# johndpope/MegaPortrait-hack

Hardware: AMD Instinct MI355X
Metric: Gbase fwd hot-slice frames/sec @512^2 (96ch 16x64x64 volume) (higher is better)
Workload: dtype f16x3 (fp32 in/out, operands split into 2 f16 halves, 3 f16 MFMAs per product, fp32 accumulate; 3x3x3 convs that fill the chip run in the F(2,3) Winograd domain along W)

## Files before the change

include/mphip.h:

```cpp
#ifndef MPHIP_H
#define MPHIP_H

#include <stddef.h>
#include <stdint.h>

#define MPHIP_RANGE_FLOATS 4100

#ifdef __cplusplus
extern "C" {
#endif

#define MPHIP_OK 0
#define MPHIP_EINVAL (-1)
#define MPHIP_ELAUNCH (-2)
#define MPHIP_EWORKSPACE (-3)

#define MPHIP_ABI_VERSION 20
int mphip_version(void);
int mphip_graph_memsets_to_kernels(void *graph, int *replaced);
int mphip_graph_memset_nodes_left(void *graph, int *left);

int mphip_build_flags(void);
const char *mphip_last_error(void);

int mphip_rt_theta(const float *rotation_deg, const float *translation, float *theta, int B, int invert,
                   void *stream);

int mphip_warp_field_compose(const float *theta, const float *em, const float *base_tbl, float *w,
                             float *rt_out, float *em_out, int B, int eD, int eH, int eW, int G,
                             void *stream);

size_t mphip_warp_workspace_bytes(int B, int D, int H, int W);
// ... 56 lines not shown
                             const float *bias, float *y, float *gn_stats, int N, int Ci, int Co, int D, int H, int W,
                             int k, int precision, int gn_groups, float gn_eps, void *workspace,
                             size_t workspace_bytes, void *stream);

int mphip_conv3d_splits(int N, int Ci, int Co, int D, int H, int W, int k, int precision);
int mphip_conv3d_fwd_split(const float *x, const float *x_range, const void *w_packed, const float *bias, float *out,
                           int N, int Ci, int Co, int D, int H, int W, int k, int precision, void *workspace,
                           size_t workspace_bytes, void *stream);

size_t mphip_groupnorm_workspace_bytes(int N, int C, int S, int G);
int mphip_groupnorm_stats(const float *x, float *stats, int N, int C, int S, int G, float eps,
                          void *workspace, size_t workspace_bytes, void *stream);
int mphip_groupnorm_apply(const float *x, const float *stats, const float *gamma, const float *beta,
                          const float *w2, const float *b2, const float *residual, float *y, float *out_range, int N,
                          int C, int D, int H, int W, int G, int relu, int tanh_, int pool2, void *stream);

int mphip_groupnorm_stats_split(const float *x, int x_splits, const float *x_bias, float *stats, int N, int C,
                                int S, int G, float eps, void *stream);
int mphip_groupnorm_apply_split(const float *x, int x_splits, const float *x_bias, const float *stats,
                                const float *gamma, const float *beta, const float *w2, const float *b2,
                                const float *residual, int res_splits, const float *res_bias, float *y,
                                float *out_range, int N, int C, int D, int H, int W, int G, int relu, int tanh_,
                                int pool2, int uD, int uH, int uW, void *stream);

int mphip_groupnorm_small_fused(const float *x, int x_splits, const float *x_bias, const float *gamma,
                                const float *beta, const float *w2, const float *b2, const float *residual,
                                int res_splits, const float *res_bias, float *y, float *stats_out, int N, int C,
                                int D, int H, int W, int G, float eps, int relu, int tanh_, int uD, int uH, int uW,
                                void *stream);

// ... 176 lines not shown
```

megaportrait-hack_amd/_lib.py:

```python
from __future__ import annotations

import ctypes
import os
import subprocess

_HERE = os.path.dirname(os.path.abspath(__file__))
LIB_PATH = os.environ.get("MPHIP_LIB", os.path.join(_HERE, "libmphip.so"))
BUILD_SCRIPT = os.path.join(_HERE, "csrc", "build.sh")

_c_float_p = ctypes.c_void_p
_i = ctypes.c_int
_sz = ctypes.c_size_t
_p = ctypes.c_void_p

class PackJob(ctypes.Structure):
    _fields_ = [("w", ctypes.c_void_p), ("wp", ctypes.c_void_p), ("like", ctypes.c_void_p), ("Co", ctypes.c_int), ("Ci", ctypes.c_int),
                ("k", ctypes.c_int), ("precision", ctypes.c_int), ("transposed", ctypes.c_int)]


SIGNATURES = {
    "mphip_version": (_i, []),
    "mphip_last_error": (ctypes.c_char_p, []),
    "mphip_rt_theta": (_i, [_p, _p, _p, _i, _i, _p]),
    "mphip_warp_field_compose": (_i, [_p, _p, _p, _p, _p, _p, _i, _i, _i, _i, _i, _p]),
# ... 23 lines not shown
    "mphip_conv3d_gn_workspace_bytes": (_sz, [_i, _i, _i, _i, _i, _i, _i, _i, _i]),
    "mphip_conv3d_gn_fwd": (_i, [_p, _p, _p, _p, _p, _p, _i, _i, _i, _i, _i, _i, _i, _i, _i, ctypes.c_float, _p, _sz, _p]),
    "mphip_conv3d_gn_table_fwd": (_i, [_p] * 12 + [_i] * 9 + [ctypes.c_float, _p, _sz, _p]),
    "mphip_conv3d_time_next_launch": (None, [_p, _p]),
    "mphip_groupnorm_affine_table": (_i, [_p, _p, _p, _p, _p, _p, _p, _i, _i, _i, _i, _p]),
    "mphip_conv3d_gnin_gn_fwd": (_i, [_p, _p, _p, _i, _p, _p, _p, _p] + [_i] * 9 + [ctypes.c_float, _p, _sz, _p]),
    "mphip_conv3d_gnin_fwd": (_i, [_p, _p, _p, _i, _p, _p, _p, _i, _i, _i, _i, _i, _i, _i, _i, _p, _sz, _p]),
    "mphip_conv3d_splits": (_i, [_i, _i, _i, _i, _i, _i, _i, _i]),
    "mphip_conv3d_fwd_split": (_i, [_p, _p, _p, _p, _p, _i, _i, _i, _i, _i, _i, _i, _i, _p, _sz, _p]),
    "mphip_groupnorm_stats_split": (_i, [_p, _i, _p, _p, _i, _i, _i, _i, ctypes.c_float, _p]),
    "mphip_groupnorm_apply_split": (_i, [_p, _i, _p, _p, _p, _p, _p, _p, _p, _i, _p, _p, _p] + [_i] * 12 + [_p]),
    "mphip_groupnorm_small_fused": (_i, [_p, _i, _p, _p, _p, _p, _p, _p, _i, _p, _p, _p] + [_i] * 6 + [ctypes.c_float] + [_i] * 5 + [_p]),
    "mphip_groupnorm_workspace_bytes": (_sz, [_i, _i, _i, _i]),
    "mphip_groupnorm_stats": (_i, [_p, _p, _i, _i, _i, _i, ctypes.c_float, _p, _sz, _p]),
    "mphip_groupnorm_apply": (_i, [_p, _p, _p, _p, _p, _p, _p, _p, _p, _i, _i, _i, _i, _i, _i, _i, _i, _i, _p]),
    "mphip_avgpool2": (_i, [_p, _p, _i, _i, _i, _i, _p]),
    "mphip_upsample_trilinear2": (_i, [_p, _p, _i, _i, _i, _i, _p]),
    "mphip_upsample_nearest": (_i, [_p, _p, _i, _i, _i, _i, _i, _i, _i, _p]),
    "mphip_upsample_trilinear": (_i, [_p, _p, _i, _i, _i, _i, _i, _i, _i, _p]),
    "mphip_upsample_trilinear_bwd": (_i, [_p, _p, _i, _i, _i, _i, _i, _i, _i, _p]),
    "mphip_add_matmul": (_i, [_p, _p, _p, _p, _p, _i, _i, _i, _i, _p]),
    "mphip_grad_prep_workspace_bytes": (_sz, [_i, _i, _i]),
    "mphip_grad_prep": (_i, [_p, _p, _p, _i, _i, _i, _p, _sz, _p]),
    "mphip_pack_conv_weight_bwd_data": (_i, [_p, _p, _i, _i, _i, _i, _p]),
    "mphip_pack_conv_weight_bwd_data_like": (_i, [_p, _p, _i, _i, _i, _i, _p, _p]),
    "mphip_conv3d_bwd_data": (_i, [_p, _p, _p, _p] + [_i] * 8 + [_p, _sz, _p]),
    "mphip_conv3d_bwd_weight_supported": (_i, [_i] * 8),
    "mphip_conv3d_bwd_weight_workspace_bytes": (_sz, [_i] * 8),
    "mphip_conv3d_bwd_weight": (_i, [_p, _p, _p, _p, _p] + [_i] * 8 + [_p, _sz, _p]),
    "mphip_groupnorm_bwd_workspace_bytes": (_sz, [_i, _i, _i]),
# ... 56 lines not shown
    "mphip_conv2d_fwd": (_i, [_p] * 7 + [_i] * 6 + [_p, _sz, _p]),
    "mphip_conv2d_cat_supported": (_i, [_i] * 6),
    "mphip_conv2d_cat_workspace_bytes": (_sz, [_i] * 6),
    "mphip_conv2d_cat_fwd": (_i, [_p, _p, _i, _p, _i] * 2 + [_p] * 5 + [_i] * 5 + [_p, _sz, _p]),
    "mphip_build_flags": (_i, []),
    "mphip_graph_memsets_to_kernels": (_i, [_p, ctypes.POINTER(ctypes.c_int)]),
    "mphip_graph_memset_nodes_left": (_i, [_p, ctypes.POINTER(ctypes.c_int)]),
    "mphip_pack_table_create": (_i, [_p, _i, ctypes.POINTER(ctypes.c_void_p)]),
    "mphip_pack_table_run": (_i, [_p, _p]),
    "mphip_pack_table_destroy": (_i, [_p]),
    "mphip_debug_dma_stream": (_i, [_p, _i, _i, _i, _i, _p, _i, _p]),
}

_lib = None

EXPECTED_ABI_VERSION = 20


def header_abi_version() -> int:
    import re

    path = os.path.join(os.path.dirname(_HERE), "include", "mphip.h")
    if not os.path.isfile(path):
        return EXPECTED_ABI_VERSION
    with open(path) as f:
        m = re.search(r"#define\s+MPHIP_ABI_VERSION\s+(\d+)", f.read())
    if m is None:
        raise RuntimeError("include/mphip.h does not define MPHIP_ABI_VERSION")
    return int(m.group(1))


# ... 44 lines not shown
```

megaportrait-hack_amd/csrc/conv3d_f16x3.hip:

```cpp
#include <stdlib.h>

#include <algorithm>


#include "mphip_ablate.h"
#include "mphip_common.h"
#include "mphip_conv.h"
#include "mphip_f16x3.h"

namespace mphip {

constexpr float X_SCALE = 16.0f;

__device__ unsigned long long g_f16x3_saturated;

#ifdef MPHIP_PROFILE_PHASES
__device__ unsigned long long g_f16x3_prof[8];
#define PROF_DECL unsigned long long pt_ = __builtin_readcyclecounter(), pa_[7] = {0, 0, 0, 0, 0, 0, 0}
#define PROF_ADD(slot) { const unsigned long long n_ = __builtin_readcyclecounter(); pa_[slot] += n_ - pt_; pt_ = n_; }
#define PROF_FLUSH if ((threadIdx.x & 63) == 0) { for (int q_ = 0; q_ < 7; ++q_) atomicAdd(&g_f16x3_prof[q_], pa_[q_]); atomicAdd(&g_f16x3_prof[7], 1ull); }
#else
#define PROF_DECL
#define PROF_ADD(slot)
#define PROF_FLUSH
// ... 621 lines not shown
        const size_t slab = (size_t)cot * nchunks + chunk;
        const size_t inner = ((size_t)kg * F16X3_COT + co) * 8 + e;
        out[slab * K1_SLAB_HALFS + inner] = hi;
        out[slab * K1_SLAB_HALFS + K1_SLAB_HALFS / 2 + inner] = lo;
    }
    if (bid == 0 && threadIdx.x == 0) {
        hdr_out[0] = 1.0f / scale;
        hdr_out[1] = scale;
    }
}
__global__ void __launch_bounds__(256) f16x3_pack_k1_kernel(const float *__restrict__ w, _Float16 *__restrict__ out, const unsigned *hdr_in,
                                                            float *__restrict__ hdr_out, int Co, int Ci, int transposed) {
    f16x3_pack_k1_body(w, out, hdr_in, hdr_out, Co, Ci, transposed, blockIdx.x, gridDim.x);
}

template <int KS, int NTT = 2>
__global__ void __launch_bounds__(KS == 1 ? 256 : 64 * KS) __attribute__((amdgpu_waves_per_eu(2)))
conv3d_k1_f16x3_kernel(const float *__restrict__ x, const _Float16 *__restrict__ wslabs, const float *__restrict__ whdr,
                       const float *__restrict__ bias, float *__restrict__ y, int N, int Ci, int Co, int DHW, unsigned x_bytes,
                       const float *__restrict__ x_range) {
    constexpr int MT = 3, NT = NTT;
    float x_scale = X_SCALE, x_unscale = 1.0f / X_SCALE;
    if (x_range) range_scale_block(x_range, x_scale, x_unscale);
    const int lane = threadIdx.x & 63, wave = threadIdx.x >> 6;
    const int j = lane & 31, kg = lane >> 5;
    const long v0 = (KS == 1 ? (long)blockIdx.x * 4 + wave : (long)blockIdx.x) * (NT * 32);
    if (v0 >= (long)N * DHW) return;
    const int n = (int)(v0 / DHW), r0 = (int)(v0 - (long)n * DHW);
    const int cot = blockIdx.y, nchunks = Ci / F16X3_KC;
    const int cps = (nchunks + KS - 1) / KS;
    const int c_begin = KS == 1 ? 0 : wave * cps, c_end = KS == 1 ? nchunks : min(nchunks, c_begin + cps);
    __amdgpu_buffer_rsrc_t rsrc = __builtin_amdgcn_make_buffer_rsrc((void *)x, 0, (int)x_bytes, 0x00020000);
    const unsigned vbase = (unsigned)((((long)n * Ci + kg * 8) * DHW + r0 + j) * 4);
    const unsigned cstride = (unsigned)DHW * 4u;
    const _Float16 *wl = wslabs + (size_t)cot * nchunks * K1_SLAB_HALFS + (kg * F16X3_COT + j) * 8;

    f32x16 acc[MT][NT];
#pragma unroll
    for (int m = 0; m < MT; ++m)
#pragma unroll
        for (int t = 0; t < NT; ++t)
#pragma unroll
            for (int q = 0; q < 16; ++q) acc[m][t][q] = 0.0f;

    unsigned sat_ = 0;
    float xv[2][NT][8];
    half8 ah[2][MT], al[2][MT];
#define K1_LOAD(set, c_)                                                                                              \
    {                                                                                                                 \
        const unsigned soff_ = (unsigned)((long)(c_) * F16X3_KC * DHW * 4);                                           \
        _Pragma("unroll") for (int t = 0; t < NT; ++t)                                                                \
            _Pragma("unroll") for (int e = 0; e < 8; ++e)                                                             \
                xv[set][t][e] = buf_load_f(rsrc, vbase + (unsigned)t * 128u + (unsigned)e * cstride, soff_);          \
        const _Float16 *ws_ = wl + (size_t)(c_) * K1_SLAB_HALFS;                                                      \
        _Pragma("unroll") for (int m = 0; m < MT; ++m) {                                                              \
            ah[set][m] = *reinterpret_cast<const half8 *>(ws_ + m * 32 * 8);                                          \
            al[set][m] = *reinterpret_cast<const half8 *>(ws_ + K1_SLAB_HALFS / 2 + m * 32 * 8);                      \
        }                                                                                                             \
    }
#define K1_MFMA(set)                                                                                                  \
    {                                                                                                                 \
        half8 bh[NT], bl[NT];                                                                                         \
        _Pragma("unroll") for (int t = 0; t < NT; ++t)                                                                \
            _Pragma("unroll") for (int e = 0; e < 8; ++e) {                                                           \
                _Float16 h, l;                                                                                        \
                const float sv = xv[set][t][e] * x_scale;                                                             \
                sat_ += !(fabsf(sv) <= F16_CLAMP);                                                                    \
                split_f16(sv, h, l);                                                                                  \
// ... 8 lines not shown
                acc[m][t] = __builtin_amdgcn_mfma_f32_32x32x16_f16(ah[set][m], bl[t], acc[m][t], 0, 0, 0);            \
        _Pragma("unroll") for (int m = 0; m < MT; ++m)                                                                \
            _Pragma("unroll") for (int t = 0; t < NT; ++t)                                                            \
                acc[m][t] = __builtin_amdgcn_mfma_f32_32x32x16_f16(ah[set][m], bh[t], acc[m][t], 0, 0, 0);            \
    }
    if (c_begin < c_end) K1_LOAD(0, c_begin)
    for (int c = c_begin; c < c_end; c += 2) {
        if (c + 1 < c_end) K1_LOAD(1, c + 1)
        K1_MFMA(0)
        if (c + 1 < c_end) {
            if (c + 2 < c_end) K1_LOAD(0, c + 2)
            K1_MFMA(1)
        }
    }
#undef K1_LOAD
#undef K1_MFMA
    const float unscale = whdr[0] * x_unscale;
    const int co0 = cot * F16X3_COT;
    if (KS == 1) {
#pragma unroll
        for (int m = 0; m < MT; ++m) {
#pragma unroll
            for (int reg = 0; reg < 16; ++reg) {
                const int co = co0 + m * 32 + (reg & 3) + 8 * (reg >> 2) + 4 * kg;
                const float bv = bias ? bias[co] : 0.0f;
                float *dv = y + ((size_t)n * Co + co) * DHW + r0 + j;
#pragma unroll
                for (int t = 0; t < NT; ++t) dv[t * 32] = acc[m][t][reg] * unscale + bv;
            }
        }
    } else {
        __shared__ float red[KS > 1 ? KS : 1][NT * 16 * 64];
#pragma unroll
        for (int m = 0; m < MT; ++m) {
#pragma unroll
            for (int t = 0; t < NT; ++t)
#pragma unroll
                for (int reg = 0; reg < 16; ++reg) red[wave][(t * 16 + reg) * 64 + lane] = acc[m][t][reg];
            __syncthreads();
            for (int q = wave; q < NT * 16; q += KS) {
                const int t = q >> 4, reg = q & 15;
                float sum = red[0][q * 64 + lane];
#pragma unroll
                for (int k = 1; k < KS; ++k) sum += red[k][q * 64 + lane];
                const int co = co0 + m * 32 + (reg & 3) + 8 * (reg >> 2) + 4 * kg;
                const float bv = bias ? bias[co] : 0.0f;
                y[((size_t)n * Co + co) * DHW + r0 + j + t * 32] = sum * unscale + bv;
            }
            __syncthreads();
        }
    }
    if (__builtin_amdgcn_ballot_w64(sat_ != 0) != 0) {
        unsigned tot = sat_;
#pragma unroll
        for (int sft = 32; sft >= 1; sft >>= 1) tot += __shfl_xor(tot, sft, 64);
        if (lane == 0) atomicAdd(&g_f16x3_saturated, (unsigned long long)tot);
    }
}

static int f16x3_k1_ksplit(const F16x3Switches &sw, int N, int Ci, int Co, int DHW) {
    if (sw.k1_ks == 1 || sw.k1_ks == 4 || sw.k1_ks == 8) return sw.k1_ks;
    const long wave_tiles = (long)N * DHW / 64 * (Co / F16X3_COT);
    const int nchunks = Ci / F16X3_KC;
    if (wave_tiles >= 1024 || nchunks < 8) return 1;
    return (wave_tiles <= 512 && nchunks >= 16) ? 8 : 4;
}

int f16x3_pack(const float *w, void *out, int Co, int Ci, int k, int transposed, const void *header_from, hipStream_t s) {
    const unsigned *hdr = (const unsigned *)out;
    if (header_from) {
        hdr = (const unsigned *)header_from;
    } else {
// ... 79 lines not shown
    const int ks = f16x3_k1_ksplit(sw, N, Ci, Co, DHW);
    const bool nt1 = ks == 1 && (sw.k1_nt >= 0 ? sw.k1_nt == 1 : waves * (Co / F16X3_COT) <= 1024);
    if (ks == 8)
        hipLaunchKernelGGL(conv3d_k1_f16x3_kernel<8>, dim3((unsigned)waves, Co / F16X3_COT), dim3(512), 0, s, x, slabs, hdr, bias, dst, N, Ci,
                           Co, DHW, xb, x_range);
    else if (ks == 4)
        hipLaunchKernelGGL(conv3d_k1_f16x3_kernel<4>, dim3((unsigned)waves, Co / F16X3_COT), dim3(256), 0, s, x, slabs, hdr, bias, dst, N, Ci,
                           Co, DHW, xb, x_range);
    else if (nt1)
        hipLaunchKernelGGL((conv3d_k1_f16x3_kernel<1, 1>), dim3((unsigned)((2 * waves + 3) / 4), Co / F16X3_COT), dim3(256), 0, s, x, slabs, hdr,
                           bias, dst, N, Ci, Co, DHW, xb, x_range);
    else
        hipLaunchKernelGGL(conv3d_k1_f16x3_kernel<1>, dim3((unsigned)((waves + 3) / 4), Co / F16X3_COT), dim3(256), 0, s, x, slabs, hdr, bias,
                           dst, N, Ci, Co, DHW, xb, x_range);
    return check_launch("conv3d_fwd(f16x3, k=1)");
}

int f16x3_launch(const F16x3Switches &sw, const F16x3Plan &p, const float *x, const void *wpacked, const float *bias, float *dst, int N, int Ci,
                 int Co, int D, int H, int W, const float *in_affine, int in_relu, const float *x_scale, hipStream_t s, const int *roi,
                 int roi_frames, int *tile_list, int roi_dilate, float *gn_part, hipEvent_t t0, hipEvent_t t1) {
    const bool wino = f16x3_is_wino(p.kernel);
    if (in_affine && Ci > p.max_gn_ci) {
        set_error("conv3d_fwd(f16x3%s): fused input GroupNorm supports Ci <= %d (got %d)", wino ? ", F(2,3)" : "", p.max_gn_ci, Ci);
        return MPHIP_EINVAL;
    }
    if ((roi && !p.tile_list) || (gn_part && !p.gn_rows)) {
        set_error("conv3d_fwd(f16x3, F(2,3), D = 2): no demand-driven tile list / GroupNorm partials in the two-frame mode");
        return MPHIP_EINVAL;
    }
    const float *hdr = (const float *)wpacked;
// ... 76 lines not shown
```

megaportrait-hack_amd/csrc/mphip_common.h:

```cpp
#pragma once
#include <hip/hip_runtime.h>
#include <stdarg.h>
#include <stdint.h>
#include <stdio.h>

#include <type_traits>

#include "../../include/mphip.h"

namespace mphip {

void set_error(const char *fmt, ...);

inline int check_launch(const char *what) {
    hipError_t e = hipGetLastError();
    if (e != hipSuccess) {
        set_error("%s: %s", what, hipGetErrorString(e));
        return MPHIP_ELAUNCH;
    }
    return MPHIP_OK;
}

#define MPHIP_REQUIRE(cond, ...)          \
    do {                                  \
// ... 119 lines not shown
    r.u = v != v ? (unsigned short)0x7FC0u : (unsigned short)((u + 0x7FFFu + ((u >> 16) & 1u)) >> 16);
    return r;
}

template <typename F>
inline int dispatch_dtype(int dtype, const char *unknown, F &&f) {
    switch (dtype) {
        case MPHIP_DTYPE_F32: return f(std::integral_constant<int, MPHIP_DTYPE_F32>{});
        case MPHIP_DTYPE_F16: return f(std::integral_constant<int, MPHIP_DTYPE_F16>{});
        case MPHIP_DTYPE_BF16: return f(std::integral_constant<int, MPHIP_DTYPE_BF16>{});
    }
    set_error("%s %d", unknown, dtype);
    return MPHIP_EINVAL;
}

__device__ __forceinline__ float sum_slabs(const float *__restrict__ x, int splits, size_t slab, size_t o) {
    float v = x[o];
    for (int z = 1; z < splits; z += 8) {
        float t[8];
#pragma unroll
        for (int k = 0; k < 8; ++k) t[k] = z + k < splits ? x[(size_t)(z + k) * slab + o] : 0.0f;
#pragma unroll
        for (int k = 0; k < 8; ++k)
            if (z + k < splits) v += t[k];
    }
    return v;
}

}
```

megaportrait-hack_amd/csrc/norm.hip:

```cpp
#include <stdlib.h>

#include "mphip_common.h"
#include "mphip_conv.h"
#include "mphip_resample.h"

namespace mphip {

constexpr int GN_CHUNK = 16384;

__device__ __forceinline__ double wave_sum(double v) {
#pragma unroll
    for (int s = 32; s >= 1; s >>= 1) v += __shfl_xor(v, s, 64);
    return v;
}


__device__ __forceinline__ void gn_span_moments(const float *__restrict__ p, size_t begin, size_t end, bool vec, float k, float &s, float &ss) {
    if (vec) {
#pragma unroll 8
        for (size_t i = begin + (size_t)threadIdx.x * 4; i < end; i += 1024) {
            float4 v = *reinterpret_cast<const float4 *>(p + i);
            v.x -= k; v.y -= k; v.z -= k; v.w -= k;
            s += (v.x + v.y) + (v.z + v.w);
            ss += (v.x * v.x + v.y * v.y) + (v.z * v.z + v.w * v.w);
// ... 169 lines not shown
        }
    }
    if (tbl.table && tbl.range) range_note_block(mbits, tbl.range, blockIdx.x, gridDim.x);
}

struct GnParams {
    const float *x, *stats, *gamma, *beta, *w2, *b2, *residual;
    float *y;
    int C, cpg;
    int relu, tanh_;
    float *range;
};

__device__ __forceinline__ float gn_value(const GnParams &p, float xv, float mean, float rstd, float g, float b,
                                          float w2, float b2, bool has2, float res, bool has_res) {
    float v = (xv - mean) * rstd * g + b;
    if (has2) v = v * w2 + b2;
    if (has_res) v += res;
    if (p.relu) v = fmaxf(v, 0.0f);
    if (p.tanh_) v = tanhf(v);
    return v;
}

template <int VW>
__global__ void __launch_bounds__(256) gn_apply_kernel(GnParams p, int S, size_t total_vec) {
    unsigned mbits = 0;
    for (size_t t = (size_t)blockIdx.x * blockDim.x + threadIdx.x; t < total_vec; t += (size_t)gridDim.x * blockDim.x) {
        const int SV = S / VW;
        size_t plane = t / SV;
        int c = (int)(plane % p.C);
        int n = (int)(plane / p.C);
        int grp = n * (p.C / p.cpg) + c / p.cpg;
        float mean = p.stats[grp * 2], rstd = p.stats[grp * 2 + 1];
// ... 904 lines not shown
```

megaportrait-hack_amd/csrc/plan.hip:

```cpp
#include <stdlib.h>
#include <string.h>

#include <string>
#include <unordered_map>
#include <vector>

#include "linspace_tables.h"
#include "mphip_common.h"

using namespace mphip;

namespace {

constexpr float GN_EPS = 1e-5f;
constexpr size_t SPLIT_CHAIN_MAX_ELEMS = 1u << 18;
constexpr int SPLIT_CHAIN_MAX_SPLITS = 16;
constexpr size_t SPLIT_CHAIN_MAX_SLAB_ELEMS = 1u << 20;
constexpr size_t STATS_SPLIT_MAX_SPAN = 65536;
constexpr size_t GN_FUSED_MAX_SPAN = 12288;
constexpr size_t ALIGN = 256;

struct Arena {
    struct Block { size_t off, size; bool free; };
    std::vector<Block> blocks;
// ... 492 lines not shown
        coords[l] = take(c, (size_t)B * p->D * p->H * p->W * 3 * sizeof(float));
        if (p->H == G && p->W == G) {
            RUN(c, mphip_warp_field_coords(theta[l].p, em[l].data.p, p->aff_base, p->lin_d, p->lin_h, p->lin_w, coords[l].p, B, em[l].d, em[l].h, em[l].w,
                                           G, p->D, c.s));
        } else {
            T5 wf = new_t5(c, B, 3, G, G, G, false);
            RUN(c, mphip_warp_field_compose(theta[l].p, em[l].data.p, p->aff_base, wf.data.p, nullptr, nullptr, B, em[l].d, em[l].h, em[l].w, G, c.s));
            RUN(c, mphip_warp_coords(wf.data.p, p->lin_d, p->lin_h, p->lin_w, coords[l].p, B, p->D, p->H, p->W, G, G, G, c.s));
            give(c, wf);
        }
        give(c, theta[l]);
        give(c, em[l]);
    }
}

template <typename Hook>
T5 resblock(Ctx &c, ResBlock &b, T5 &x, bool pool_after, Hook hook) {
    ConvOut identity = b.identity ? as_convout(x) : conv3d_split(c, x, b.shortcut, 0);
    ConvOut y = conv3d_split(c, x, b.conv1, 32, &b.gn1, &b.conv2);
    hook();
    ensure_stats(c, y, 32);
    ConvOut y2;
    if (y.splits == 1 && gn_in_conv_ok(c, y, b.conv2)) {
        y2 = conv3d_gn_in(c, y, b.gn1, 32, b.conv2, 32);
        give(c, y);
    } else {
        T5 a = groupnorm_apply(c, y, b.gn1, 32, nullptr, true, false, false, 1, 1, 1);
        give(c, y);
        y2 = conv3d_split(c, a, b.conv2, 32);
        give(c, a);
    }
    ensure_stats(c, y2, 32);
    T5 out = groupnorm_apply(c, y2, b.gn2, 32, &identity, true, false, pool_after, 1, 1, 1);
    give(c, y2);
    if (!b.identity) give(c, identity);
    give(c, x);
    return out;
}

struct Roi {
    const int *box = nullptr;
    bool on = false;
    int tile[3] = {0, 0, 0};
};

T5 upsample2(Ctx &c, T5 &x, const Roi *roi = nullptr) {
    T5 y;
    y.n = x.n; y.c = x.c; y.d = 2 * x.d; y.h = 2 * x.h; y.w = 2 * x.w;
// ... 507 lines not shown
```

megaportrait-hack_amd/model.py:

```python
from __future__ import annotations

import logging
import os

import torch
import torch.nn as nn
import torch.nn.functional as F

from . import autograd as ag
from . import ops

COMPRESS_DIM = 512
_C2D_EARLY = os.environ.get("MPHIP_C2D_EARLY", "0") == "1"


def _f32(*tensors):
    out = tuple(t.float() if isinstance(t, torch.Tensor) and t.is_floating_point() and t.dtype != torch.float32 else t
                for t in tensors)
    return out[0] if len(out) == 1 else out


def _autocast_policy(fn):
    import functools

# ... 377 lines not shown
        return ag.groupnorm(y, self.gn2, residual=identity, relu=True)

    def forward(self, x, _pool_after: bool = False, _after_conv1=None):
        out = self._forward(x, _pool_after, _after_conv1)
        if self.upsample:
            out = _upsample_trilinear(out, self.scale_factors)
        return out

    def _forward(self, x, _pool_after: bool = False, _after_conv1=None):
        x = _f32(x)
        if ag.needs_grad(self, x):
            y = self._forward_train(x)
            if _after_conv1 is not None:
                _after_conv1()
            return ag.AvgPool2Fn.apply(y) if _pool_after else y
        identity = x if isinstance(self.shortcut, nn.Identity) else ops.conv3d_split(x, _packs.get(self.shortcut))
        y = ops.conv3d_split(x, _packs.get(self.conv1), gn_groups=32, gn_eps=self.gn1.eps)
        if _after_conv1 is not None:
            _after_conv1()
        st = ops.groupnorm_stats(y, 32, self.gn1.eps)
        pc2 = _packs.get(self.conv2)
        if y.splits == 1 and ops.gn_in_conv_ok(y.shape, pc2):
            y2, st2 = ops.conv3d_gn_in(y.data, st, self.gn1.weight, self.gn1.bias, 32, pc2, out_gn_groups=32,
                                       out_gn_eps=self.gn2.eps)
            y = ops.ConvOut(y2, 1, None, y.shape, st2, 32)
        else:
            a = ops.groupnorm_apply(y, st, self.gn1.weight, self.gn1.bias, 32, relu=True)
            y = ops.conv3d_split(a, pc2, gn_groups=32, gn_eps=self.gn2.eps)
        st = ops.groupnorm_stats(y, 32, self.gn2.eps)
        return ops.groupnorm_apply(y, st, self.gn2.weight, self.gn2.bias, 32, residual=identity, relu=True,
                                   pool2=_pool_after)


class G3d(_ModelDtype, nn.Module):

    def __init__(self, in_channels):
        super().__init__()
        self.downsampling = nn.Sequential(
            ResBlock3D(in_channels, 96), nn.AvgPool3d(kernel_size=2, stride=2),
            ResBlock3D(96, 192), nn.AvgPool3d(kernel_size=2, stride=2),
            ResBlock3D(192, 384), nn.AvgPool3d(kernel_size=2, stride=2),
            ResBlock3D(384, 768),
        )
        self.upsampling = nn.Sequential(
# ... 593 lines not shown
```

megaportrait-hack_amd/ops.py:

```python
from __future__ import annotations

import ctypes
from typing import Optional, Tuple

import os as _os

import torch

from . import _lib

_P = ctypes.c_void_p


def _ptr(t: Optional[torch.Tensor]):
    return None if t is None else _P(t.data_ptr())


def _stream():
    return _P(torch.cuda.current_stream().cuda_stream)


def _req(t: torch.Tensor, name: str, dtype=torch.float32) -> torch.Tensor:
    if not isinstance(t, torch.Tensor) or not t.is_cuda:
        raise RuntimeError(f"{name}: expected a CUDA tensor (the HIP path has no CPU fallback), got "
# ... 688 lines not shown
    rng = new_range(xt.device) if _RANGES_ENABLED else None
    if general:
        xb = x.bias if isinstance(x, ConvOut) else None
        rb = residual.bias if isinstance(residual, ConvOut) else None
        _lib.check(lib.mphip_groupnorm_apply_split(_ptr(xt), xs, _ptr(xb), _ptr(stats), _ptr(gamma), _ptr(beta), _ptr(w2), _ptr(b2),
                                                   _ptr(rt), rs, _ptr(rb), _ptr(y), _ptr(rng), n, c, d, h, w, groups, int(relu),
                                                   int(tanh), int(pool2), up[0], up[1], up[2], _stream()),
                   "mphip_groupnorm_apply_split")
    else:
        _lib.check(lib.mphip_groupnorm_apply(_ptr(xt), _ptr(stats), _ptr(gamma), _ptr(beta), _ptr(w2), _ptr(b2), _ptr(rt),
                                             _ptr(y), _ptr(rng), n, c, d, h, w, groups, int(relu), int(tanh), int(pool2),
                                             _stream()), "mphip_groupnorm_apply")
    return tag_range(y, rng)


_GN_FUSED_MAX_SPAN = 12288


_GN_SMALL_ENABLED = _os.environ.get("MPHIP_GN_SMALL", "1") != "0"


def groupnorm_fused_ok(x, groups: int) -> bool:
    if not _GN_SMALL_ENABLED:
        return False
    shape = x.shape if isinstance(x, ConvOut) else tuple(x.shape)
    n, c, d, h, w = shape
    return (c // groups) * d * h * w <= _GN_FUSED_MAX_SPAN


def groupnorm_small(x, gamma, beta, groups: int, eps: float = 1e-5, w2=None, b2=None, residual=None, relu=False,
# ... 520 lines not shown
```

Measured before the change: 3215.

## Fuse 1x1x1 shortcut conv into the final GroupNorm apply epilogue

Adds a kernel that computes the 1x1x1 shortcut convolution with f16x3 MFMAs and, in its epilogue, applies GroupNorm to the conv2 output, adds the shortcut result as the residual, applies ReLU and optionally the 2x average pool, then writes the final block output. This removes the separate shortcut conv launch and the write and re-read of the identity tensor. In exchange the conv kernel epilogue gains extra global loads of y2 (including split-slab summation), more shared-memory parameters and higher register pressure. The pooling variant remaps voxel lanes so that pooled cells reduce through shuffles.

Result: no change. 3241, median of 6 (+0.8%).

```diff
diff --git a/include/mphip.h b/include/mphip.h
--- a/include/mphip.h
+++ b/include/mphip.h
@@ -15,7 +15,7 @@
 #define MPHIP_ELAUNCH (-2)
 #define MPHIP_EWORKSPACE (-3)
 
-#define MPHIP_ABI_VERSION 20
+#define MPHIP_ABI_VERSION 21
 int mphip_version(void);
 int mphip_graph_memsets_to_kernels(void *graph, int *replaced);
 int mphip_graph_memset_nodes_left(void *graph, int *left);
@@ -102,6 +102,12 @@
 int mphip_groupnorm_apply(const float *x, const float *stats, const float *gamma, const float *beta,
                           const float *w2, const float *b2, const float *residual, float *y, float *out_range, int N,
                           int C, int D, int H, int W, int G, int relu, int tanh_, int pool2, void *stream);
+
+int mphip_shortcut_gn_apply_supported(int N, int Ci, int Co, int D, int H, int W, int pool2);
+int mphip_shortcut_gn_apply(const float *x, const float *x_range, const void *w_packed, const float *bias, const float *y2,
+                            int y2_splits, const float *y2_bias, const float *stats, const float *gamma, const float *beta,
+                            const float *w2, const float *b2, float *y, float *out_range, int N, int Ci, int Co, int D, int H,
+                            int W, int G, int pool2, void *stream);
 
 int mphip_groupnorm_stats_split(const float *x, int x_splits, const float *x_bias, float *stats, int N, int C,
                                 int S, int G, float eps, void *stream);
diff --git a/megaportrait-hack_amd/_lib.py b/megaportrait-hack_amd/_lib.py
--- a/megaportrait-hack_amd/_lib.py
+++ b/megaportrait-hack_amd/_lib.py
@@ -61,6 +61,8 @@
     "mphip_groupnorm_workspace_bytes": (_sz, [_i, _i, _i, _i]),
     "mphip_groupnorm_stats": (_i, [_p, _p, _i, _i, _i, _i, ctypes.c_float, _p, _sz, _p]),
     "mphip_groupnorm_apply": (_i, [_p, _p, _p, _p, _p, _p, _p, _p, _p, _i, _i, _i, _i, _i, _i, _i, _i, _i, _p]),
+    "mphip_shortcut_gn_apply_supported": (_i, [_i] * 7),
+    "mphip_shortcut_gn_apply": (_i, [_p, _p, _p, _p, _p, _i, _p, _p, _p, _p, _p, _p, _p, _p] + [_i] * 8 + [_p]),
     "mphip_avgpool2": (_i, [_p, _p, _i, _i, _i, _i, _p]),
     "mphip_upsample_trilinear2": (_i, [_p, _p, _i, _i, _i, _i, _p]),
     "mphip_upsample_nearest": (_i, [_p, _p, _i, _i, _i, _i, _i, _i, _i, _p]),
@@ -147,7 +149,7 @@
 
 _lib = None
 
-EXPECTED_ABI_VERSION = 20
+EXPECTED_ABI_VERSION = 21
 
 
 def header_abi_version() -> int:
diff --git a/megaportrait-hack_amd/csrc/conv3d_f16x3.hip b/megaportrait-hack_amd/csrc/conv3d_f16x3.hip
--- a/megaportrait-hack_amd/csrc/conv3d_f16x3.hip
+++ b/megaportrait-hack_amd/csrc/conv3d_f16x3.hip
@@ -659,25 +659,112 @@
     f16x3_pack_k1_body(w, out, hdr_in, hdr_out, Co, Ci, transposed, blockIdx.x, gridDim.x);
 }
 
-template <int KS, int NTT = 2>
-__global__ void __launch_bounds__(KS == 1 ? 256 : 64 * KS) __attribute__((amdgpu_waves_per_eu(2)))
-conv3d_k1_f16x3_kernel(const float *__restrict__ x, const _Float16 *__restrict__ wslabs, const float *__restrict__ whdr,
-                       const float *__restrict__ bias, float *__restrict__ y, int N, int Ci, int Co, int DHW, unsigned x_bytes,
-                       const float *__restrict__ x_range) {
+struct K1Fuse {
+    const float *y2, *y2_bias, *stats, *gamma, *beta, *w2, *b2;
+    float *out, *range;
+    size_t slab;
+    int splits, cpg, H, W;
+};
+constexpr int K1_PRM = 8;
+
+__device__ __forceinline__ float k1_sum_slabs(const float *__restrict__ x, int splits, size_t slab, size_t o) {
+    float v = x[o];
+#pragma nounroll
+    for (int z = 1; z < splits; ++z) v += x[(size_t)z * slab + o];
+    return v;
+}
+
+template <int NT, int EPI>
+__device__ __forceinline__ unsigned k1_fuse_emit(const K1Fuse &f, const float *__restrict__ prm, int ch, const float (&acc)[NT], const float (&yv)[NT],
+                                                 float unscale, size_t plane, int DHW, const int (&rv)[NT], int cellq, int lane, unsigned bm) {
+    const float mean = prm[0 * F16X3_COT + ch], rstd = prm[1 * F16X3_COT + ch], g = prm[2 * F16X3_COT + ch], b = prm[3 * F16X3_COT + ch];
+    const float w2 = prm[4 * F16X3_COT + ch], b2 = prm[5 * F16X3_COT + ch], xb = prm[6 * F16X3_COT + ch], bv = prm[7 * F16X3_COT + ch];
+    const bool has2 = f.w2 != nullptr;
+    float v[NT];
+#pragma unroll
+    for (int t = 0; t < NT; ++t) {
+        float sv = acc[t] * unscale + bv;
+        float xv = yv[t];
+        if (f.splits > 1) {
+            xv = xv + xb;
+            sv = sv + 0.0f;
+        }
+        v[t] = fmaxf(gn_norm_value(xv, mean, rstd, g, b, w2, b2, has2, sv, true), 0.0f);
+    }
+    unsigned mbits = 0;
+    if (EPI == 2) {
+        float s = 0.0f;
+#pragma unroll
+        for (int t = 0; t < NT; ++t) {
+            s += v[t];
+            s += __shfl_xor(v[t], 1, 64);
+            s += __shfl_xor(v[t], (int)bm, 64);
+            s += __shfl_xor(v[t], (int)(bm | 1u), 64);
+        }
+        if ((lane & (int)(bm | 1u)) == 0) {
+            f.out[plane * (size_t)(DHW >> 3) + cellq] = s / 8.0f;
+            mbits = range_bits(s / 8.0f);
+        }
+    } else {
+#pragma unroll
+        for (int t = 0; t < NT; ++t) {
+            f.out[plane * (size_t)DHW + rv[t]] = v[t];
+            mbits = max(mbits, range_bits(v[t]));
+        }
+    }
+    return mbits;
+}
+
+template <int KS, int NTT, int EPI>
+__device__ __forceinline__ void k1_f16x3_body(const float *__restrict__ x, const _Float16 *__restrict__ wslabs, const float *__restrict__ whdr,
+                                              const float *__restrict__ bias, float *__restrict__ y, int N, int Ci, int Co, int DHW, unsigned x_bytes,
+                                              const float *__restrict__ x_range, const K1Fuse &f) {
     constexpr int MT = 3, NT = NTT;
+    static_assert(EPI != 2 || NT == 2, "the pooling epilogue holds the two depths of a pooled cell in the two column tiles");
     float x_scale = X_SCALE, x_unscale = 1.0f / X_SCALE;
     if (x_range) range_scale_block(x_range, x_scale, x_unscale);
     const int lane = threadIdx.x & 63, wave = threadIdx.x >> 6;
     const int j = lane & 31, kg = lane >> 5;
     const long v0 = (KS == 1 ? (long)blockIdx.x * 4 + wave : (long)blockIdx.x) * (NT * 32);
-    if (v0 >= (long)N * DHW) return;
-    const int n = (int)(v0 / DHW), r0 = (int)(v0 - (long)n * DHW);
+    const bool active = v0 < (long)N * DHW;
+    if (EPI == 0 && !active) return;
+    const int n = active ? (int)(v0 / DHW) : 0, r0 = active ? (int)(v0 - (long)n * DHW) : 0;
     const int cot = blockIdx.y, nchunks = Ci / F16X3_KC;
     const int cps = (nchunks + KS - 1) / KS;
-    const int c_begin = KS == 1 ? 0 : wave * cps, c_end = KS == 1 ? nchunks : min(nchunks, c_begin + cps);
+    const int c_begin = KS == 1 ? 0 : wave * cps, c_end = !active ? c_begin : KS == 1 ? nchunks : min(nchunks, c_begin + cps);
     __amdgpu_buffer_rsrc_t rsrc = __builtin_amdgcn_make_buffer_rsrc((void *)x, 0, (int)x_bytes, 0x00020000);
-    const unsigned vbase = (unsigned)((((long)n * Ci + kg * 8) * DHW + r0 + j) * 4);
     const unsigned cstride = (unsigned)DHW * 4u;
+    int rv[NT], cellq = 0;
+    unsigned bm = 16;
+#pragma unroll
+    for (int t = 0; t < NT; ++t) rv[t] = r0 + j + t * 32;
+    if (EPI == 2) {
+        const int oW = f.W >> 1, oH = f.H >> 1;
+        int cw = (j >> 1) & 7, hb = j >> 4;
+        if (oW < 8) { cw = ((j >> 4) << 2) | ((j >> 1) & 3); hb = (j >> 3) & 1; bm = 8; }
+        cellq = (r0 >> 3) + cw;
+        const int ow = cellq % oW, oh = (cellq / oW) % oH, od = cellq / (oW * oH);
+#pragma unroll
+        for (int t = 0; t < NT; ++t) rv[t] = ((2 * od + t) * f.H + 2 * oh + hb) * f.W + 2 * ow + (j & 1);
+    }
+    const unsigned vbase = (unsigned)((((long)n * Ci + kg * 8) * DHW + rv[0]) * 4);
+    __shared__ float prm_[EPI ? (KS == 1 ? 4 : 1) : 1][EPI ? K1_PRM * F16X3_COT : 1];
+    const float *prm = prm_[KS == 1 && EPI ? wave : 0];
+    if (EPI) {
+        for (int i = KS == 1 ? lane : (int)threadIdx.x; i < F16X3_COT && active; i += KS == 1 ? 64 : KS * 64) {
+            float *q = prm_[KS == 1 ? wave : 0] + i;
+            const int co = cot * F16X3_COT + i, grp = n * (Co / f.cpg) + co / f.cpg;
+            q[0 * F16X3_COT] = f.stats[grp * 2];
+            q[1 * F16X3_COT] = f.stats[grp * 2 + 1];
+            q[2 * F16X3_COT] = f.gamma[co];
+            q[3 * F16X3_COT] = f.beta[co];
+            q[4 * F16X3_COT] = f.w2 ? f.w2[co] : 1.0f;
+            q[5 * F16X3_COT] = f.w2 ? f.b2[co] : 0.0f;
+            q[6 * F16X3_COT] = (f.splits > 1 && f.y2_bias) ? f.y2_bias[co] : 0.0f;
+            q[7 * F16X3_COT] = bias ? bias[co] : 0.0f;
+        }
+        __syncthreads();
+    }
     const _Float16 *wl = wslabs + (size_t)cot * nchunks * K1_SLAB_HALFS + (kg * F16X3_COT + j) * 8;
 
     f32x16 acc[MT][NT];
@@ -691,12 +778,13 @@
     unsigned sat_ = 0;
     float xv[2][NT][8];
     half8 ah[2][MT], al[2][MT];
+#define K1_VOX(t) (EPI == 2 ? (unsigned)(rv[t] - rv[0]) * 4u : (unsigned)(t) * 128u)
 #define K1_LOAD(set, c_)                                                                                              \
     {                                                                                                                 \
         const unsigned soff_ = (unsigned)((long)(c_) * F16X3_KC * DHW * 4);                                           \
         _Pragma("unroll") for (int t = 0; t < NT; ++t)                                                                \
             _Pragma("unroll") for (int e = 0; e < 8; ++e)                                                             \
-                xv[set][t][e] = buf_load_f(rsrc, vbase + (unsigned)t * 128u + (unsigned)e * cstride, soff_);          \
+                xv[set][t][e] = buf_load_f(rsrc, vbase + K1_VOX(t) + (unsigned)e * cstride, soff_);                   \
         const _Float16 *ws_ = wl + (size_t)(c_) * K1_SLAB_HALFS;                                                      \
         _Pragma("unroll") for (int m = 0; m < MT; ++m) {                                                              \
             ah[set][m] = *reinterpret_cast<const half8 *>(ws_ + m * 32 * 8);                                          \
@@ -735,10 +823,38 @@
         }
     }
 #undef K1_LOAD
+#undef K1_VOX
 #undef K1_MFMA
     const float unscale = whdr[0] * x_unscale;
     const int co0 = cot * F16X3_COT;
-    if (KS == 1) {
+    unsigned mbits = 0;
+    if (EPI && KS == 1) {
+        if (active) {
+#pragma unroll
+            for (int m = 0; m < MT; ++m) {
+                float yv[16][NT];
+                if (f.splits == 1) {
+#pragma unroll
+                    for (int reg = 0; reg < 16; ++reg)
+#pragma unroll
+                        for (int t = 0; t < NT; ++t)
+                            yv[reg][t] = f.y2[((size_t)n * Co + co0 + m * 32 + (reg & 3) + 8 * (reg >> 2) + 4 * kg) * DHW + rv[t]];
+                }
+#pragma unroll
+                for (int reg = 0; reg < 16; ++reg) {
+                    const int ch = m * 32 + (reg & 3) + 8 * (reg >> 2) + 4 * kg;
+                    float a[NT];
+#pragma unroll
+                    for (int t = 0; t < NT; ++t) a[t] = acc[m][t][reg];
+                    if (f.splits > 1) {
+#pragma unroll
+                        for (int t = 0; t < NT; ++t) yv[reg][t] = k1_sum_slabs(f.y2, f.splits, f.slab, ((size_t)n * Co + co0 + ch) * DHW + rv[t]);
+                    }
+                    mbits = max(mbits, k1_fuse_emit<NT, EPI>(f, prm, ch, a, yv[reg], unscale, (size_t)n * Co + co0 + ch, DHW, rv, cellq, lane, bm));
+                }
+            }
+        }
+    } else if (KS == 1) {
 #pragma unroll
         for (int m = 0; m < MT; ++m) {
 #pragma unroll
@@ -759,6 +875,23 @@
 #pragma unroll
                 for (int reg = 0; reg < 16; ++reg) red[wave][(t * 16 + reg) * 64 + lane] = acc[m][t][reg];
             __syncthreads();
+            if (EPI) {
+                for (int reg = wave; reg < 16 && active; reg += KS) {
+                    const int ch = m * 32 + (reg & 3) + 8 * (reg >> 2) + 4 * kg;
+                    const size_t plane = (size_t)n * Co + co0 + ch;
+                    float a[NT], yv[NT];
+#pragma unroll
+                    for (int t = 0; t < NT; ++t) {
+                        const int q = t * 16 + reg;
+                        a[t] = red[0][q * 64 + lane];
+#pragma unroll
+                        for (int k = 1; k < KS; ++k) a[t] += red[k][q * 64 + lane];
+                        const size_t o = plane * DHW + rv[t];
+                        yv[t] = f.splits > 1 ? k1_sum_slabs(f.y2, f.splits, f.slab, o) : f.y2[o];
+                    }
+                    mbits = max(mbits, k1_fuse_emit<NT, EPI>(f, prm, ch, a, yv, unscale, plane, DHW, rv, cellq, lane, bm));
+                }
+            } else
             for (int q = wave; q < NT * 16; q += KS) {
                 const int t = q >> 4, reg = q & 15;
                 float sum = red[0][q * 64 + lane];
@@ -777,6 +910,23 @@
         for (int sft = 32; sft >= 1; sft >>= 1) tot += __shfl_xor(tot, sft, 64);
         if (lane == 0) atomicAdd(&g_f16x3_saturated, (unsigned long long)tot);
     }
+    if (EPI && f.range) range_note_block(mbits, f.range, blockIdx.y * gridDim.x + blockIdx.x, gridDim.x * gridDim.y);
+}
+
+template <int KS, int NTT = 2>
+__global__ void __launch_bounds__(KS == 1 ? 256 : 64 * KS) __attribute__((amdgpu_waves_per_eu(2)))
+conv3d_k1_f16x3_kernel(const float *__restrict__ x, const _Float16 *__restrict__ wslabs, const float *__restrict__ whdr,
+                       const float *__restrict__ bias, float *__restrict__ y, int N, int Ci, int Co, int DHW, unsigned x_bytes,
+                       const float *__restrict__ x_range) {
+    k1_f16x3_body<KS, NTT, 0>(x, wslabs, whdr, bias, y, N, Ci, Co, DHW, x_bytes, x_range, K1Fuse{});
+}
+
+template <int KS, int NTT, int POOL>
+__global__ void __launch_bounds__(KS == 1 ? 256 : 64 * KS) __attribute__((amdgpu_waves_per_eu(2)))
+shortcut_gn_apply_kernel(const float *__restrict__ x, const _Float16 *__restrict__ wslabs, const float *__restrict__ whdr,
+                         const float *__restrict__ bias, int N, int Ci, int Co, int DHW, unsigned x_bytes, const float *__restrict__ x_range,
+                         K1Fuse f) {
+    k1_f16x3_body<KS, NTT, 1 + POOL>(x, wslabs, whdr, bias, nullptr, N, Ci, Co, DHW, x_bytes, x_range, f);
 }
 
 static int f16x3_k1_ksplit(const F16x3Switches &sw, int N, int Ci, int Co, int DHW) {
@@ -886,6 +1036,54 @@
         hipLaunchKernelGGL(conv3d_k1_f16x3_kernel<1>, dim3((unsigned)((waves + 3) / 4), Co / F16X3_COT), dim3(256), 0, s, x, slabs, hdr, bias,
                            dst, N, Ci, Co, DHW, xb, x_range);
     return check_launch("conv3d_fwd(f16x3, k=1)");
+}
+
+static bool shortcut_gn_geometry(const F16x3Switches &sw, int N, int Ci, int Co, int D, int H, int W, int pool2, int &ks, bool &nt1, dim3 &grid) {
+    if (!f16x3_supported(sw, N, Ci, Co, D, H, W, 1)) return false;
+    if (pool2 && !(D % 2 == 0 && H % 2 == 0 && (W == 8 || W % 16 == 0))) return false;
+    const int DHW = D * H * W;
+    const long waves = (long)N * DHW / 64;
+    ks = f16x3_k1_ksplit(sw, N, Ci, Co, DHW);
+    nt1 = !pool2 && ks == 1 && (sw.k1_nt >= 0 ? sw.k1_nt == 1 : waves * (Co / F16X3_COT) <= 1024);
+    grid = dim3((unsigned)(ks > 1 ? waves : nt1 ? (2 * waves + 3) / 4 : (waves + 3) / 4), Co / F16X3_COT);
+    return (long)grid.x * grid.y <= (long)RANGE_MAX_PARTS;
+}
+
+extern "C" int mphip_shortcut_gn_apply_supported(int N, int Ci, int Co, int D, int H, int W, int pool2) {
+    int ks;
+    bool nt1;
+    dim3 grid;
+    return N > 0 && Ci > 0 && Co > 0 && D > 0 && H > 0 && W > 0 && shortcut_gn_geometry(f16x3_switches(), N, Ci, Co, D, H, W, pool2, ks, nt1, grid);
+}
+
+extern "C" int mphip_shortcut_gn_apply(const float *x, const float *x_range, const void *w_packed, const float *bias, const float *y2, int y2_splits,
+                                       const float *y2_bias, const float *stats, const float *gamma, const float *beta, const float *w2,
+                                       const float *b2, float *y, float *out_range, int N, int Ci, int Co, int D, int H, int W, int G, int pool2,
+                                       void *stream) {
+    MPHIP_REQUIRE(x && x_range && w_packed && y2 && stats && gamma && beta && y, "shortcut_gn_apply: null pointer");
+    MPHIP_REQUIRE(N > 0 && Ci > 0 && Co > 0 && D > 0 && H > 0 && W > 0 && G > 0 && Co % G == 0 && y2_splits >= 1, "shortcut_gn_apply: bad dims");
+    MPHIP_REQUIRE((w2 == nullptr) == (b2 == nullptr), "shortcut_gn_apply: w2/b2 must both be set or both NULL");
+    int ks;
+    bool nt1;
+    dim3 grid;
+    MPHIP_REQUIRE(shortcut_gn_geometry(f16x3_switches(), N, Ci, Co, D, H, W, pool2, ks, nt1, grid),
+                  "shortcut_gn_apply: shape not supported (query mphip_shortcut_gn_apply_supported)");
+    const int DHW = D * H * W;
+    const float *hdr = (const float *)w_packed;
+    const _Float16 *slabs = (const _Float16 *)((const char *)w_packed + 16);
+    const unsigned xb = (unsigned)((size_t)N * Ci * DHW * 4);
+    const K1Fuse f{y2, y2_bias, stats, gamma, beta, w2, b2, y, out_range, (size_t)N * Co * DHW, y2_splits, Co / G, H, W};
+    hipStream_t s = (hipStream_t)stream;
+#define MPHIP_SGA(KS_, NT_, POOL_)                                                                                                           \
+    hipLaunchKernelGGL((shortcut_gn_apply_kernel<KS_, NT_, POOL_>), grid, dim3(KS_ == 1 ? 256 : 64 * KS_), 0, s, x, slabs, hdr, bias, N, Ci, Co, \
+                       DHW, xb, x_range, f)
+    if (ks == 8) { if (pool2) MPHIP_SGA(8, 2, 1); else MPHIP_SGA(8, 2, 0); }
+    else if (ks == 4) { if (pool2) MPHIP_SGA(4, 2, 1); else MPHIP_SGA(4, 2, 0); }
+    else if (nt1) MPHIP_SGA(1, 1, 0);
+    else if (pool2) MPHIP_SGA(1, 2, 1);
+    else MPHIP_SGA(1, 2, 0);
+#undef MPHIP_SGA
+    return check_launch("shortcut_gn_apply");
 }
 
 int f16x3_launch(const F16x3Switches &sw, const F16x3Plan &p, const float *x, const void *wpacked, const float *bias, float *dst, int N, int Ci,
diff --git a/megaportrait-hack_amd/csrc/mphip_common.h b/megaportrait-hack_amd/csrc/mphip_common.h
--- a/megaportrait-hack_amd/csrc/mphip_common.h
+++ b/megaportrait-hack_amd/csrc/mphip_common.h
@@ -157,6 +157,14 @@
     return MPHIP_EINVAL;
 }
 
+__device__ __forceinline__ float gn_norm_value(float xv, float mean, float rstd, float g, float b, float w2, float b2, bool has2, float res,
+                                               bool has_res) {
+    float v = (xv - mean) * rstd * g + b;
+    if (has2) v = v * w2 + b2;
+    if (has_res) v += res;
+    return v;
+}
+
 __device__ __forceinline__ float sum_slabs(const float *__restrict__ x, int splits, size_t slab, size_t o) {
     float v = x[o];
     for (int z = 1; z < splits; z += 8) {
diff --git a/megaportrait-hack_amd/csrc/norm.hip b/megaportrait-hack_amd/csrc/norm.hip
--- a/megaportrait-hack_amd/csrc/norm.hip
+++ b/megaportrait-hack_amd/csrc/norm.hip
@@ -207,9 +207,7 @@
 
 __device__ __forceinline__ float gn_value(const GnParams &p, float xv, float mean, float rstd, float g, float b,
                                           float w2, float b2, bool has2, float res, bool has_res) {
-    float v = (xv - mean) * rstd * g + b;
-    if (has2) v = v * w2 + b2;
-    if (has_res) v += res;
+    float v = gn_norm_value(xv, mean, rstd, g, b, w2, b2, has2, res, has_res);
     if (p.relu) v = fmaxf(v, 0.0f);
     if (p.tanh_) v = tanhf(v);
     return v;
diff --git a/megaportrait-hack_amd/csrc/plan.hip b/megaportrait-hack_amd/csrc/plan.hip
--- a/megaportrait-hack_amd/csrc/plan.hip
+++ b/megaportrait-hack_amd/csrc/plan.hip
@@ -530,9 +530,15 @@
     }
 }
 
+bool shortcut_fused_ok(const Ctx &c, const T5 &x, const ConvW &sc, bool pool2) {
+    static const bool fuse = !(getenv("MPHIP_FUSE_SHORTCUT") && getenv("MPHIP_FUSE_SHORTCUT")[0] == '0');
+    return fuse && c.p->precision == 1 && sc.k == 1 && mphip_shortcut_gn_apply_supported(x.n, sc.ci, sc.co, x.d, x.h, x.w, pool2) != 0;
+}
+
 template <typename Hook>
 T5 resblock(Ctx &c, ResBlock &b, T5 &x, bool pool_after, Hook hook) {
-    ConvOut identity = b.identity ? as_convout(x) : conv3d_split(c, x, b.shortcut, 0);
+    const bool fuse = !b.identity && shortcut_fused_ok(c, x, b.shortcut, pool_after);
+    ConvOut identity = b.identity || fuse ? as_convout(x) : conv3d_split(c, x, b.shortcut, 0);
     ConvOut y = conv3d_split(c, x, b.conv1, 32, &b.gn1, &b.conv2);
     hook();
     ensure_stats(c, y, 32);
@@ -547,7 +553,16 @@
         give(c, a);
     }
     ensure_stats(c, y2, 32);
-    T5 out = groupnorm_apply(c, y2, b.gn2, 32, &identity, true, false, pool_after, 1, 1, 1);
+    T5 out;
+    if (fuse) {
+        const float *xr = range_for(c, x);
+        const void *wp = packed(c, b.shortcut, 1);
+        out = pool_after ? new_t5(c, x.n, y2.t.c, x.d / 2, x.h / 2, x.w / 2, true) : new_t5(c, x.n, y2.t.c, x.d, x.h, x.w, true);
+        RUN(c, mphip_shortcut_gn_apply(x.data.p, xr, wp, b.shortcut.b, y2.t.data.p, y2.splits, y2.bias, y2.stats.p, b.gn2.gw, b.gn2.gb, b.gn2.w2,
+                                       b.gn2.b2, out.data.p, out.range.p, x.n, b.shortcut.ci, b.shortcut.co, x.d, x.h, x.w, 32, pool_after, c.s));
+    } else {
+        out = groupnorm_apply(c, y2, b.gn2, 32, &identity, true, false, pool_after, 1, 1, 1);
+    }
     give(c, y2);
     if (!b.identity) give(c, identity);
     give(c, x);
diff --git a/megaportrait-hack_amd/model.py b/megaportrait-hack_amd/model.py
--- a/megaportrait-hack_amd/model.py
+++ b/megaportrait-hack_amd/model.py
@@ -415,7 +415,8 @@
             if _after_conv1 is not None:
                 _after_conv1()
             return ag.AvgPool2Fn.apply(y) if _pool_after else y
-        identity = x if isinstance(self.shortcut, nn.Identity) else ops.conv3d_split(x, _packs.get(self.shortcut))
+        fuse = not isinstance(self.shortcut, nn.Identity) and ops.shortcut_gn_apply_ok(x.shape, _packs.get(self.shortcut), _pool_after)
+        identity = x if fuse or isinstance(self.shortcut, nn.Identity) else ops.conv3d_split(x, _packs.get(self.shortcut))
         y = ops.conv3d_split(x, _packs.get(self.conv1), gn_groups=32, gn_eps=self.gn1.eps)
         if _after_conv1 is not None:
             _after_conv1()
@@ -429,6 +430,8 @@
             a = ops.groupnorm_apply(y, st, self.gn1.weight, self.gn1.bias, 32, relu=True)
             y = ops.conv3d_split(a, pc2, gn_groups=32, gn_eps=self.gn2.eps)
         st = ops.groupnorm_stats(y, 32, self.gn2.eps)
+        if fuse:
+            return ops.shortcut_gn_apply(x, _packs.get(self.shortcut), y, st, self.gn2.weight, self.gn2.bias, 32, pool2=_pool_after)
         return ops.groupnorm_apply(y, st, self.gn2.weight, self.gn2.bias, 32, residual=identity, relu=True,
                                    pool2=_pool_after)
 
diff --git a/megaportrait-hack_amd/ops.py b/megaportrait-hack_amd/ops.py
--- a/megaportrait-hack_amd/ops.py
+++ b/megaportrait-hack_amd/ops.py
@@ -726,6 +726,37 @@
     return tag_range(y, rng)
 
 
+_FUSE_SHORTCUT = _os.environ.get("MPHIP_FUSE_SHORTCUT", "1") != "0"
+
+
+def shortcut_gn_apply_ok(x_shape, pc: "PackedConv", pool2: bool = False) -> bool:
+    if not _FUSE_SHORTCUT or _default_precision != 1 or not _RANGES_ENABLED or pc.k != 1:
+        return False
+    n, ci, d, h, w = x_shape
+    return bool(_lib.load().mphip_shortcut_gn_apply_supported(n, ci, pc.co, d, h, w, int(pool2)))
+
+
+def shortcut_gn_apply(x: torch.Tensor, pc: "PackedConv", y2, stats, gamma, beta, groups: int, w2=None, b2=None,
+                      pool2: bool = False) -> torch.Tensor:
+    x = _req(x, "x")
+    lib = _lib.load()
+    ys = y2.splits if isinstance(y2, ConvOut) else 1
+    yt = _req(y2.data if isinstance(y2, ConvOut) else y2, "y2")
+    yb = y2.bias if isinstance(y2, ConvOut) else None
+    n, ci, d, h, w = x.shape
+    if tuple(y2.shape[-5:]) != (n, pc.co, d, h, w) or ci != pc.ci:
+        raise RuntimeError("shortcut_gn_apply: shape mismatch")
+    gamma, beta = _req(gamma.detach(), "gamma"), _req(beta.detach(), "beta")
+    if w2 is not None:
+        w2, b2 = _req(w2.detach(), "w2").reshape(-1), _req(b2.detach(), "b2").reshape(-1)
+    y = torch.empty((n, pc.co, d // 2, h // 2, w // 2) if pool2 else (n, pc.co, d, h, w), dtype=torch.float32, device=x.device)
+    rng = new_range(x.device) if _RANGES_ENABLED else None
+    _lib.check(lib.mphip_shortcut_gn_apply(_ptr(x), _ptr(_range_for(x)), _ptr(pc.packed(1)), _ptr(pc.bias), _ptr(yt), ys, _ptr(yb),
+                                           _ptr(stats), _ptr(gamma), _ptr(beta), _ptr(w2), _ptr(b2), _ptr(y), _ptr(rng), n, ci, pc.co,
+                                           d, h, w, groups, int(pool2), _stream()), "mphip_shortcut_gn_apply")
+    return tag_range(y, rng)
+
+
 _GN_FUSED_MAX_SPAN = 12288
 
 
```
